# sashajenner/honours

Hardware: AMD Instinct MI355X
Metric: raw-signal MB/s (compress+decompress) (higher is better)
Workload: dtype u16

## Files before the change

### honours_amd/csrc/press_exsplit.hip

```cpp

#include "press_chunk.h"

namespace ph {

__device__ __forceinline__ void quarter_zd(const int16_t *in, uint32_t n, uint32_t ws, int lane, int q,
					   uint4 (&z)[CK], uint32_t &ored)
{
#pragma unroll
	for (int k = 0; k < CK; k++) {
		const uint32_t i0 = ws + k * SUB + lane * 8;
		z[k] = make_uint4(0, 0, 0, 0);
		if (i0 < n)
			z[k] = ld16_stream(in + i0);
	}
	uint32_t carry = 0;
	if (ws > 0 && ws < n)
		carry = (uint32_t) (uint16_t) in[ws - 1] << 16;
	uint32_t o = 0;
	const s16x2 qq = { (short) q, (short) q };
#pragma unroll
	for (int k = 0; k < CK; k++) {
		const uint32_t i0 = ws + k * SUB + lane * 8;
		uint32_t r[4] = { z[k].x, z[k].y, z[k].z, z[k].w };
		if (i0 + 8 > n) {
// ... 422 lines not shown
		unsigned long long mask = __ballot(valid && zv <= 255u);
		while (mask && got < nb) {
			const int l = 63 - __builtin_clzll(mask);
			const uint32_t e = enc[(uint32_t) __builtin_amdgcn_readlane((int) zv, l)];
			const uint32_t len = e >> 24;
			acc = (acc << len) | (e & 0xFFFFFFu);
			got += len;
			mask &= ~(1ull << l);
		}
		pos = pos > 64 ? pos - 64 : 0;
	}
	return got >= nb ? (acc >> (got - nb)) & ((1u << nb) - 1u) : acc;
}


__global__ __launch_bounds__(CWG, HENC_WAVES) void k_huff_encode_chunked(BatchArgs a)
{
	__shared__ uint32_t enc[257];
	__shared__ uint32_t stg_all[4][HSTG];

	enc[threadIdx.x] = a.huff->enc[threadIdx.x];
	if (threadIdx.x == 0)
		enc[256] = 0;
	for (uint32_t i = threadIdx.x; i < 4u * HSTG; i += CWG)
		(&stg_all[0][0])[i] = 0;
	__syncthreads();
	const uint32_t t = blockIdx.x;
	if (t >= uni(a.ctl->nchunks))
		return;
	const int lane = threadIdx.x & 63;
// ... 17 lines not shown
	const uint64_t before = uni64(cb->before);
	if (w == 0 && last) {
		const uint64_t bits = before + q0 + q1 + q2 + q3;
		const uint64_t total = (uint64_t) head + (bits + 7) / 8;
		const uint32_t nbt = (uint32_t) bits & 7u;
		if (total <= cap && nbt) {
			const uint32_t tb = huff_tail_bits(in, n, nbt, enc, lane);
			if (lane == 0)
				payload[bits >> 3] = (uint8_t) tb;
		}
		if (lane == 0)
			a.out_len[d.read] = total <= cap ? total : CFAIL64;
	}
	const uint32_t mybits = w == 0 ? q0 : w == 1 ? q1 : w == 2 ? q2 : q3;
	const uint64_t Bq = before + (w > 0 ? q0 : 0u) + (w > 1 ? q1 : 0u) + (w > 2 ? q2 : 0u);
	if (ws >= n || !mybits || (uint64_t) head + (Bq + mybits + 7) / 8 > cap)
		return;
	const uint32_t nb = (uint32_t) Bq & 7u;
	if (nb) {
		const uint32_t tb = huff_tail_bits(in, ws, nb, enc, lane);
		if (lane == 0)
			stg[0] = tb;
	}
	uint8_t *g = payload + (Bq >> 3);
	uint32_t fill = nb;
	wave_lds_sync();
	static_assert(CK % HENC_G == 0, "a quarter is a whole number of groups");
	uint4 raw[HENC_G];
#pragma unroll
	for (int gi = 0; gi < HENC_G; gi++)
		raw[gi] = sub_load(in, n, ws + gi * SUB + lane * 8);
	uint32_t carry = ws > 0 ? (uint32_t) (uint16_t) in[ws - 1] << 16 : 0u;
// ... 17 lines not shown
			const uint32_t sub0 = ws + (kg + gi) * SUB;
			if (sub0 >= n)
				break;
			const uint32_t i0 = sub0 + lane * 8;
			const uint4 z = sub_zd(cur[gi], n, i0, carry);
			const uint32_t zz[4] = { z.x, z.y, z.z, z.w };
			uint32_t e[8];
			uint32_t lb = 0;
			if (sub0 != 0 && sub0 + SUB <= n && !__ballot(((z.x | z.y | z.z | z.w) & 0xFF00FF00u) != 0)) {
#pragma unroll
				for (int h = 0; h < 8; h++) {
					e[h] = enc[(zz[h >> 1] >> (16 * (h & 1))) & 0xFFu];
					lb += e[h] >> 24;
				}
			} else {
				const uint32_t lowm = low_mask(z, i0, n);
#pragma unroll
				for (int h = 0; h < 8; h++) {
					e[h] = enc[((lowm >> h) & 1u) ? ((zz[h >> 1] >> (16 * (h & 1))) & 0xFFu) : 256u];
					lb += e[h] >> 24;
				}
			}
			const uint32_t inc = wave_incl_scan_dpp(lb);
			const uint32_t tot = (uint32_t) __builtin_amdgcn_readlane((int) inc, 63);
			uint32_t pos = fill + inc - lb;
			if (lb <= 64) {
				uint64_t acc = 0;
				uint32_t o = 0;
#pragma unroll
				for (int h = 0; h < 8; h++) {
// ... 39 lines not shown
			fill = total & 31u;
			wave_lds_sync();
		}
	}
	if (lane == 0) {
		const uint32_t v = stg[0];
		for (uint32_t b = 0; b < (fill >> 3); b++)
			g[b] = (uint8_t) (v >> (8 * b));
	}
}


__global__ __launch_bounds__(256) void k_chunk_prep_meta(const uint64_t *off, const uint64_t *in_off,
							 const ReadMeta *meta, uint32_t nreads, ChunkDesc *chunks,
							 uint64_t *gran, ChunkCtl *ctl, uint32_t max_chunks,
							 uint32_t *out_n, const uint32_t *hread, const uint32_t *ex_pos)
{
	const uint32_t r = blockIdx.x * 256 + threadIdx.x;
	uint32_t n = 0, nch = 0;
	if (r < nreads && !meta[r].status) {
		const uint32_t nex = meta[r].nex;
		n = 1u + meta[r].nlow + nex;
		nch = (n + CHUNK - 1) / CHUNK;
		if (hread && (hread[2 * r + 1] & HUF_FUSED))
			nch = 0;
		else if (hread && nex && (uint64_t) ex_pos[off[r] + nex - 1] + 1 > (uint64_t) meta[r].nlow + nex)
			n = nch = 0;
	}
	const uint32_t inc = scan32(nch, threadIdx.x & 63);
	uint32_t base = 0;
	if ((threadIdx.x & 63) == 63 && inc)
		base = atomicAdd(&ctl->nchunks, inc);
	base = (uint32_t) __builtin_amdgcn_readlane((int) base, 63);
	const uint32_t first = base + inc - nch;
	if (r >= nreads)
		return;
	out_n[r] = n ? n : CFAIL32;
	for (uint32_t j = 0; j < nch && first + j < max_chunks; j++) {
		ChunkDesc d;
		d.sig_off = off[r];
		d.out_base = in_off[r];
		d.n = n;
// ... 63 lines not shown
			if (i == 0) {
				z = zd0;
			} else if (i - 1 == nextpos) {
				z = val[e] & 0xFFFFu;
				e++;
				nextpos = e < nex ? pos[e] : 0xFFFFFFFFu;
			} else {
				z = l < nlow ? low[l] : 0u;
				l++;
			}
			v[h >> 1] |= z << (16 * (h & 1));
		}
	}
}

template <bool HUFF>
__global__ __launch_bounds__(CWG) void k_low_decode_chunked(DecodeArgs a)
{
	__shared__ uint32_t s_ticket;
	__shared__ uint32_t s_wsum[4];
	__shared__ uint32_t s_sbase;
	__shared__ uint16_t s_xl[4][CK][64];
	__shared__ uint32_t s_sub[4][CK];
	__shared__ uint32_t s_cnt[4][CK];
	__shared__ uint32_t s_km[4];

	const int lane = threadIdx.x & 63;
	const int w = (int) uni(threadIdx.x >> 6);
#ifdef DEC_STAMPS
	const uint64_t t_start = __builtin_amdgcn_s_memtime();
#endif
// ... 18 lines not shown
	const ChunkU d = load_chunk(a.chunks + t);
	const uint32_t n = d.n;
	const uint32_t first = d.j * CHUNK;
	const bool last = first + CHUNK >= n;
	const ReadMeta *m = a.meta + d.read;
	const uint32_t nex = uni(m->nex), nlow = uni(m->nlow), zd0 = uni(m->zd0);
	const int q = (int) uni(m->q);
	const uint32_t *pos = a.ex_pos + d.sig_off;
	const uint32_t *val = a.ex_val + d.sig_off;
	const uint8_t *low = HUFF ? a.low + d.sig_off : a.in + d.out_base + uni(m->hdr) + uni(m->seclen);
	int16_t *out = a.sig + d.sig_off;
	const uint32_t ws = first + w * WAVE_SAMPLES;
	const uint32_t nsub = ws >= n ? 0u : min((uint32_t) CK, (n - ws + SUB - 1) / SUB);
	const uint32_t live = (1u << nsub) - 1u;

	const ChunkDesc *dp = a.chunks + t;
	const uint32_t c0 = uni(dp->ecnt[0]), c1 = uni(dp->ecnt[1]), c2 = uni(dp->ecnt[2]), c3 = uni(dp->ecnt[3]);
	const uint32_t ew = w == 0 ? c0 : w == 1 ? c1 : w == 2 ? c2 : c3;
	const uint32_t e_lo = (uint32_t) uni64(dp->ebefore) + (w > 0 ? c0 : 0u) + (w > 1 ? c1 : 0u) + (w > 2 ? c2 : 0u);
	if (nsub) {
		const uint32_t e_hi = e_lo + ew;
		for (uint32_t e = e_lo + lane; e < e_hi; e += 64) {
			const uint32_t k = (pos[e] + 1 - ws) / SUB;
			atomicAdd(&s_cnt[w][k], 1u);
			atomicOr(&s_km[w], 1u << k);
		}
	}
	wave_lds_sync();
	uint32_t kmask = uni(s_km[w]);
	if (ws == 0)
		kmask |= 1u;
	if ((n & 7) && n > ws && n - ws <= WAVE_SAMPLES)
		kmask |= 1u << ((n - 1 - ws) / SUB);
	if (lane < CK) {
// ... 157 lines not shown
static void ex_pass_a(const BatchArgs &a, ExEnt ent, hipStream_t s)
{
	n_pass_a++;
	if (ent == ENT_SHUFF)
		hipLaunchKernelGGL((k_ex_scan_chunked<false, true>), dim3(a.max_chunks), dim3(CWG), 0, s, a);
	else
		hipLaunchKernelGGL((k_ex_scan_chunked<false>), dim3(a.max_chunks), dim3(CWG), 0, s, a);
}

void launch_ex_encode_chunked(const BatchArgs &a, ExFmt fmt, ExEnt ent, hipStream_t s)
{
	if (!a.nreads || !a.max_chunks)
		return;
	ex_encode_prep(a, s);
	ex_pass_a(a, ent, s);
	ex_encode_lists(a, fmt, s);
	ex_encode_streams(a, fmt, ent, s);
}

void ex_packed_sizes(const BatchArgs &a, ExFmt fmt, ExEnt ent, uint64_t *need, hipStream_t s)
{
	const ExStage &st = EX_STAGES[ent];
	launch_ex_sizes(a, fmt, ent, need, s);
	if (st.pay != PAY_STAGED)
		return;
	hipLaunchKernelGGL(k_low_encode_chunked<false>, dim3(a.max_chunks), dim3(CWG), 0, s, a);
	st.press(a, need, s);
}

void ex_packed_streams(const BatchArgs &a, ExFmt fmt, ExEnt ent, hipStream_t s)
{
// ... 2 lines not shown
		return ex_encode_streams(a, fmt, ent, s);
	launch_ex_section(a, fmt, ent, s);
	ktime_begin(0, s);
	st.write_sized(a, s);
	ktime_end(0, s);
}

void launch_ex_encode_packed(const BatchArgs &a, ExFmt fmt, ExEnt ent, const PackArgs &pk, int phases, hipStream_t s)
{
	if (!a.nreads || !a.max_chunks)
		return;
	if (phases & PACK_SIZE) {
		(void) hipMemsetAsync(pk.slot, 0, ((size_t) a.nreads + 1) * 8, s);
		ex_encode_prep(a, s);
		ex_pass_a(a, ent, s);
		ex_encode_lists(a, fmt, s);
		ex_packed_sizes(a, fmt, ent, pk.need, s);
		if (pk.layout) {
			launch_pack_scan(pk, a.nreads, s);
			launch_pack_patch(a, pk.slot, s);
		}
	}
	if (phases & PACK_WRITE)
		ex_packed_streams(a, fmt, ent, s);
}

void launch_ex_prefix_sizes(const BatchArgs &a, ExFmt fmt, ExEnt ent, uint64_t *need, hipStream_t s)
{
	if (!a.nreads || !a.max_chunks || !EX_STAGES[ent].sizes_only)
		return;
	ex_encode_prep(a, s);
	ex_pass_a(a, ent, s);
	ex_encode_lists(a, fmt, s);
	launch_ex_sizes(a, fmt, ent, need, s);
	hipLaunchKernelGGL(k_low_encode_chunked<false>, dim3(a.max_chunks), dim3(CWG), 0, s, a);
	EX_STAGES[ent].press(a, need, s);
}

void ex_encode_lists(const BatchArgs &a, ExFmt fmt, hipStream_t s)
{
	if (fmt == EXF_EXZD) {
		hipLaunchKernelGGL(k_ex_redo_flag, dim3((a.nreads + 255) / 256), dim3(256), 0, s, a);
		hipLaunchKernelGGL((k_ex_scan_chunked<true>), dim3(a.max_chunks), dim3(CWG), 0, s, a);
	}
	hipLaunchKernelGGL(k_ex_prefix, dim3((a.nreads + 3) / 4), dim3(256), 0, s, a, fmt == EXF_EXZD ? 1 : 0);
	hipLaunchKernelGGL(k_ex_list, dim3((a.max_chunks + 3) / 4), dim3(CWG), 0, s, a);
}

void launch_low_encode(const BatchArgs &a, uint64_t *, hipStream_t s)
{
	if (a.zhist)
		hipLaunchKernelGGL(k_low_encode_chunked<true>, dim3(a.max_chunks), dim3(CWG), 0, s, a);
	else
		hipLaunchKernelGGL(k_low_encode_chunked<false>, dim3(a.max_chunks), dim3(CWG), 0, s, a);
}
void launch_shuff_encode(const BatchArgs &a, uint64_t *, hipStream_t s)
{
	hipLaunchKernelGGL(k_huff_encode_chunked, dim3(a.max_chunks), dim3(CWG), 0, s, a);
}

void ex_encode_streams(const BatchArgs &a, ExFmt fmt, ExEnt ent, hipStream_t s)
{
	const ExStage &st = EX_STAGES[ent];
	launch_ex_section(a, fmt, ent, s);
	if (st.low_tmp)
		hipLaunchKernelGGL(k_low_encode_chunked<false>, dim3(a.max_chunks), dim3(CWG), 0, s, a);
	ktime_begin(0, s);
	st.press(a, nullptr, s);
	ktime_end(0, s);
}

void launch_ex_decode_chunked(const DecodeArgs &a, ExFmt fmt, ExEnt ent, hipStream_t s)
{
	const bool huff = EX_STAGES[ent].depress != nullptr;
	if (!a.nreads || !a.max_chunks)
		return;
	launch_ex_parse_huff(a, fmt, ent, s);
	hipLaunchKernelGGL(k_chunk_prep_meta, dim3((a.nreads + 255) / 256), dim3(256), 0, s, a.off, a.in_off,
			   a.meta, a.nreads, a.chunks, a.gran, a.ctl, a.max_chunks, a.out_n,
			   ent == ENT_SHUFF ? (const uint32_t *) a.hread : (const uint32_t *) nullptr, a.ex_pos);
	hipLaunchKernelGGL(k_ex_ranks, dim3((a.max_chunks * 8 + 255) / 256), dim3(256), 0, s, a);
	if (!huff)
		ktime_begin(1, s);
	if (ent == ENT_SHUFF) {
		const uint32_t grid = a.max_chunks < 1024u ? a.max_chunks : 1024u;
		hipLaunchKernelGGL((k_low_decode_chunked<true>), dim3(grid), dim3(CWG), 0, s, a);
	} else if (huff) {
		hipLaunchKernelGGL((k_low_decode_chunked<true>), dim3(a.max_chunks), dim3(CWG), 0, s, a);
	} else {
		hipLaunchKernelGGL((k_low_decode_chunked<false>), dim3(a.max_chunks), dim3(CWG), 0, s, a);
	}
	if (!huff)
		ktime_end(1, s);
}

}
```

### honours_amd/csrc/press_huffman.hip

```cpp

#include "press_internal.h"
#include "press_packed.h"
#include "press_wave.h"
#include <cstddef>
#include <type_traits>

namespace ph {

#ifdef HUF_STAMPS
__device__ unsigned long long g_hstamp[32];
#define HSTAMP_DECL                                             \
	unsigned long long hs_t = __builtin_amdgcn_s_memtime(); \
	unsigned long long hs_acc[8] = { 0, 0, 0, 0, 0, 0, 0, 0 }
#define HSTAMP(i)                                                              \
	do {     \
		__builtin_amdgcn_sched_barrier(0);                             \
		const unsigned long long hs_n = __builtin_amdgcn_s_memtime(); \
		hs_acc[(i) & 7] += hs_n - hs_t;                                \
		hs_t = hs_n;                                                   \
		__builtin_amdgcn_sched_barrier(0);                             \
	} while (0)
#define HSTAMP_FLUSH(base)                                                     \
	do {                                                                   \
		if ((threadIdx.x & 63) == 0)                                   \
// ... 159 lines not shown
}

__device__ __forceinline__ int32_t unzz8(uint32_t z) { return (int32_t) (z >> 1) ^ -(int32_t) (z & 1u); }

typedef __attribute__((address_space(3))) const uint32_t *lds_cu32p;
typedef __attribute__((address_space(3))) const uint16_t *lds_cu16p;
typedef __attribute__((address_space(3))) const uint8_t *lds_cu8p;
typedef __attribute__((address_space(3))) uint8_t *lds_u8p;

struct LenTabs {
	alignas(16) uint32_t alut[1 << HUF_LUT_BITS];
	alignas(16) uint16_t flut[1 << HUF_LUT_BITS];
	alignas(16) uint16_t l2ld[HUF_L2_ENTRIES];
};

template <bool TRIE, int S = 64>
__device__ __forceinline__ uint32_t len_scan(const uint32_t *col_, const LenTabs *tabs, const HuffDev *hd, uint32_t start,
					     uint32_t lim, uint32_t nb, uint32_t &cnt, uint32_t &dsum)
{
	const lds_cu32p col = (lds_cu32p) col_;
	const lds_cu32p alut = (lds_cu32p) tabs->alut;
	const lds_cu16p flut = (lds_cu16p) tabs->flut;
	const lds_cu16p l2ld = (lds_cu16p) tabs->l2ld;
	bool bad = start == HEND;
	uint32_t L = lim < nb ? lim : nb;
	if (bad)
		L = 0;
	auto long_ld = [&](uint32_t e, uint32_t wnd) -> uint32_t {
		if (TRIE && e == 0xFFFFFFFFu) {
			const uint32_t t = trie_code(hd, wnd);
			return t ? (((t >> 24) & 31u) | (((uint32_t) unzz8(t & 0xFFu) & 0xFFu) << 8)) : 0u;
		}
		const uint32_t v = l2ld[(e & 0xFFFu) + ((wnd >> HUF_LUT_BITS) & ((1u << ((e >> 12) & 15u)) - 1u))];
		return v == 0xFFFFu ? 0u : v;
	};
	constexpr uint32_t PB = 30;
	const lds_cu32p colm = col - S;
	uint32_t A = (bad ? 0u : start) + PB;
// ... 55 lines not shown
		const bool fits = pp + tot <= L;
		const bool cut = !fits && pp + len1 > nb;
		if (act && !fail && !cut) {
			p += fits ? tot : len1;
			c += fits ? n : 1u;
			d += fits ? dall : d1;
		}
		if (act && (fail || cut)) {
			bad = true;
			L = 0;
		}
	}
	cnt = c;
	dsum = (uint32_t) d & 0xFFFFu;
	return bad ? HEND : (p >= nb && p < lim ? HEND : p);
}



#ifndef HUF_SYNC_PER_CU
#define HUF_SYNC_PER_CU 2
#endif
#ifndef HUF_RUNUP_EIGHTHS
#define HUF_RUNUP_EIGHTHS 4
#endif
constexpr int WGS = 1024;
constexpr int SYNC_S = 64;

__device__ __forceinline__ uint32_t pack_rec(uint32_t f, uint32_t c, uint32_t d)
{
// ... 258 lines not shown
				atomicAdd(reinterpret_cast<unsigned long long *>(a.hwave + (uint64_t) k * (HT / 64) + (tid >> 6)),
					  (dd << 32) + (unsigned long long) dc);
			if (e8 != old_e) {
				a.hend[g] = (uint8_t) e8;
				const bool more = tid + 1 < HT || !(dp->t_last >> 31);
				next = more && (uint64_t) tid * OWN + OWN < nbits_t;
			}
		}
		list_push(out_list, out_cnt, a.hlist_cap, next, (uint32_t) g + 1, lane);
		if (last && next)
			atomicMin(&a.hmin[dp->read], (uint32_t) g + 1);
	}
}

template <int RU, bool TRIE>
__global__ __launch_bounds__(64) void k_huf_serial(DecodeArgs a)
{
	constexpr int OWN = HufGeo<RU>::OWN, NDW = HufGeo<RU>::NDW, NCOL = HufGeo<RU>::NCOL;
	struct Lds {
		LenTabs tabs;
		uint32_t img[NCOL * 64 + 64];
	};
	__shared__ __attribute__((aligned(16))) Lds lds;
	auto &img = lds.img;

	const uint32_t r = blockIdx.x;
	const uint32_t g0 = uniform(a.hmin[r]);
	if (g0 == 0xFFFFFFFFu)
		return;
	const uint32_t lane = threadIdx.x;
	const uint32_t k0 = uniform(a.hread[2 * r]), nt = uniform(a.hread[2 * r + 1]);
	load_len_tables(a.huff, &lds.tabs, 64);
	uint32_t *col = img + lane;
	const uint64_t gend = (uint64_t) (k0 + nt) * HT;
	for (uint64_t g = g0; g < gend; g++) {
		const uint32_t k = (uint32_t) (g / HT), tid = (uint32_t) (g % HT);
		const HufTile *dp = a.htiles + k;
		const uint32_t nbits_t = uniform(dp->nbits);
		if ((uint64_t) tid * OWN >= nbits_t)
			break;
		const uint32_t pe = uniform((uint32_t) __hip_atomic_load(a.hend + g - 1, __ATOMIC_RELAXED, __HIP_MEMORY_SCOPE_AGENT));
		const uint32_t rec = uniform(__hip_atomic_load(a.hrec + g, __ATOMIC_RELAXED, __HIP_MEMORY_SCOPE_AGENT));
		if ((rec & 0xFFu) == pe)
			continue;
		wave_lds_sync();
		if (lane == 0)
			col_load<NDW>(col, a.in + dp->src, (int32_t) tid * (OWN / 8), 0, (int32_t) ((nbits_t + 7) >> 3));
		wave_lds_sync();
		uint32_t c2, d2;
		const uint32_t e2 = len_scan<TRIE>(col, &lds.tabs, a.huff, (lane || pe == R_END) ? HEND : pe, OWN,
					     clamp_nb((int64_t) nbits_t - (int64_t) tid * OWN), c2, d2);
		if (lane == 0) {
			a.hrec[g] = pack_rec(pe == R_END ? HEND : pe, c2, d2);
			atomicAdd(reinterpret_cast<unsigned long long *>(a.hwave + (uint64_t) k * (HT / 64) + (tid >> 6)),
				  ((unsigned long long) ((d2 - (rec >> 16)) & 0xFFFFu) << 32) +
					  (unsigned long long) (long long) (int32_t) (c2 - ((rec >> 8) & 0xFFu)));
			__hip_atomic_store(a.hend + g, (uint8_t) (e2 == HEND ? R_END : e2 - OWN), __ATOMIC_RELAXED, __HIP_MEMORY_SCOPE_AGENT);
		}
		__builtin_amdgcn_fence(__ATOMIC_RELEASE, "agent");
	}
}

__device__ __forceinline__ uint32_t unzz16(uint32_t z) { return ((z >> 1) ^ (0u - (z & 1u))) & 0xFFFFu; }

__device__ __forceinline__ void keys_below2(const uint32_t *pos, uint32_t nex, uint32_t ka, uint32_t kb, uint32_t &ea, uint32_t &eb)
{
	uint32_t la = 0, lb = 0;
	for (uint32_t step = nex ? 1u << (31 - __builtin_clz(nex)) : 0u; step; step >>= 1) {
		const uint32_t ia = la + step - 1, ib = lb + step - 1;
		const uint32_t pa = ia < nex ? pos[ia] : 0u, pb = ib < nex ? pos[ib] : 0u;
		if (ia < nex && pa - ia < ka)
			la += step;
		if (ib < nex && pb - ib < kb)
			lb += step;
	}
	ea = la;
	eb = lb;
}

template <int RU>
__global__ __launch_bounds__(HT) void k_huf_chain(DecodeArgs a)
{
	constexpr uint32_t UB = 64 * HufGeo<RU>::OWN / 8;
	constexpr uint32_t UPT = HT / 64;
	__shared__ uint32_t s_w[HT / 64], s_wd[HT / 64];
	__shared__ unsigned long long s_cum;
	__shared__ uint32_t s_stop, s_refuse;

	const uint32_t r = blockIdx.x;
	const uint32_t tid = threadIdx.x;
	const uint32_t k0 = uniform(a.hread[2 * r]), nt = uniform(a.hread[2 * r + 1]);
	if (!nt)
		return;
	const uint32_t nu = nt * UPT;
	const uint2 *hw = a.hwave + (uint64_t) k0 * UPT;
	if (tid == 0) {
		s_cum = 0;
		s_stop = 0xFFFFFFFFu;
		s_refuse = 0;
	}
	__syncthreads();
	{
		uint64_t c = 0;
		for (uint32_t u = tid; u < nu; u += HT)
			c += hw[u].x;
		if (c)
			atomicAdd(&s_cum, (unsigned long long) c);
	}
// ... 118 lines not shown
			uint4 *d = reinterpret_cast<uint4 *>(a.hunit + (uint64_t) k0 * UPT + u);
			d[0] = make_uint4((uint32_t) src, (uint32_t) (src >> 32) | (bz << 16), (uint32_t) o0, (uint32_t) (o0 >> 32));
			d[1] = make_uint4(L0, quota | (nbyc << 14) | ((q & 15u) << 26) | (fused ? 1u << 30 : 0u), Ea, Eb - Ea);
		}
		cum += total;
		dcum += dtotal;
		__syncthreads();
	}
	static_assert(HUF_U_QUOTA >= 64u * 255u, "a unit's quota");
	if (tid == 0) {
		a.meta[r].nlow = nlow;
		if (refused)
			a.meta[r].status = 1;
		if (fused)
			a.hread[2 * r + 1] = nt | HUF_FUSED;
	}
}


constexpr uint32_t EMIT_STG = 4096;

template <bool TRIE>
__device__ __forceinline__ void emit_codes(const uint32_t *col_, const uint32_t *lut_, const uint16_t *lut2_,
					   const HuffDev *hd, uint32_t p, uint32_t nmine, uint8_t *wp_)
{
	const lds_cu32p col = (lds_cu32p) col_;
	const lds_cu8p lut = (lds_cu8p) lut_;
	const lds_cu16p lut2 = (lds_cu16p) lut2_;
	auto long_entry = [&](uint32_t e, uint32_t wnd) -> uint32_t {
		if (TRIE && e == 0xFFFFFFFFu) {
// ... 564 lines not shown
namespace ph {
#endif

constexpr int HUF_FIX_LAUNCHES = HUF_FIX_ROUNDS;

template <int RU, bool TRIE>
static void run_huff_decode(const DecodeArgs &a, hipStream_t s)
{
	const uint32_t nt = a.max_htiles ? a.max_htiles : 1;
	const uint32_t ngs = (nt * (HT / 64) + WGS / 64 - 1) / (WGS / 64);
	const uint32_t grid = ngs < HUF_SYNC_PER_CU * 256u ? ngs : HUF_SYNC_PER_CU * 256u;
	const uint32_t nge = (nt * (HT / 64) + WGE / 64 - 1) / (WGE / 64);
	const uint32_t ge = nge < EMIT_PER_CU * 256u ? nge : EMIT_PER_CU * 256u;
	hipLaunchKernelGGL((k_huf_sync<RU, TRIE>), dim3(grid), dim3(WGS), 0, s, a);
	hipLaunchKernelGGL(k_huf_list, dim3((nt * (HT / 64) + LIST_WG - 1) / LIST_WG), dim3(LIST_WG), 0, s, a);
	for (int round = 0; round < HUF_FIX_LAUNCHES; round++)
		hipLaunchKernelGGL((k_huf_fix<RU, TRIE>), dim3(FIX_WG >= 1024 ? 512 : FIX_WG >= 512 ? 768 : 1280), dim3(FIX_WG), 0, s, a, round, round + 1 == HUF_FIX_LAUNCHES ? 1 : 0);
	hipLaunchKernelGGL((k_huf_serial<RU, TRIE>), dim3(a.nreads), dim3(64), 0, s, a);
	hipLaunchKernelGGL(k_huf_chain<RU>, dim3(a.nreads), dim3(HT), 0, s, a);
	hipLaunchKernelGGL((k_huf_emit<RU, TRIE>), dim3(ge), dim3(WGE), 0, s, a);
}

template <int RU>
static void run_huff_decode_t(const DecodeArgs &a, bool trie, hipStream_t s)
{
	if (trie)
		run_huff_decode<RU, true>(a, s);
	else
		run_huff_decode<RU, false>(a, s);
}

void launch_huff_decode(const DecodeArgs &a0, hipStream_t s)
{
	const bool trie = (a0.huf_minlen & HUF_NEEDS_TRIE) != 0;
// ... 14 lines not shown
```

### honours_amd/csrc/press_internal.h

```cpp
#pragma once

#include <hip/hip_runtime.h>
#include <stdint.h>

namespace ph {

enum ExFmt : int {
	EXF_VBE21 = 0,
	EXF_VBBE21 = 1,
	EXF_VBSBE21 = 2,
	EXF_VBSSE21 = 3,
	EXF_EXZD = 4
};
enum ExEnt : int {
	ENT_PLAIN,
	ENT_SHUFF,
	ENT_RC,
	ENT_RCC,
	ENT_RCM,
	ENT_CDF,
	ENT_RICE,
	ENT_DHUF,
	ENT_COUNT
};
// ... 476 lines not shown
	{ ENT_RCM, PAY_CODER, launch_rcm_encode, launch_rcm_decode, true, false, nullptr },
	{ ENT_CDF, PAY_CODER, launch_cdf_encode, launch_cdf_decode, true, false, nullptr },
	{ ENT_RICE, PAY_STAGED, launch_rice_encode, launch_rice_decode, true, true, launch_rice_write_sized },
	{ ENT_DHUF, PAY_STAGED, launch_dhuf_encode, launch_dhuf_decode, true, true, launch_dhuf_write_sized },
};
constexpr bool ex_stages_in_order()
{
	for (int i = 0; i < ENT_COUNT; i++)
		if (EX_STAGES[i].id != i)
			return false;
	return true;
}
static_assert(ex_stages_in_order(), "EX_STAGES[i].id == i");

void ex_encode_prep(const BatchArgs &a, hipStream_t s);
void ex_encode_lists(const BatchArgs &a, ExFmt fmt, hipStream_t s);
void ex_encode_streams(const BatchArgs &a, ExFmt fmt, ExEnt ent, hipStream_t s);
void launch_ex_encode_chunked(const BatchArgs &a, ExFmt fmt, ExEnt ent, hipStream_t s);
void launch_ex_encode_packed(const BatchArgs &a, ExFmt fmt, ExEnt ent, const PackArgs &pk, int phases, hipStream_t s);
void ex_packed_sizes(const BatchArgs &a, ExFmt fmt, ExEnt ent, uint64_t *need, hipStream_t s);
void ex_packed_streams(const BatchArgs &a, ExFmt fmt, ExEnt ent, hipStream_t s);
void launch_ex_prefix_sizes(const BatchArgs &a, ExFmt fmt, ExEnt ent, uint64_t *need, hipStream_t s);
void launch_ex_decode_chunked(const DecodeArgs &a, ExFmt fmt, ExEnt ent, hipStream_t s);
void launch_ex_section(const BatchArgs &a, ExFmt fmt, ExEnt ent, hipStream_t s);
void launch_ex_sizes(const BatchArgs &a, ExFmt fmt, ExEnt ent, uint64_t *need, hipStream_t s);
void launch_ex_parse_huff(const DecodeArgs &a, ExFmt fmt, ExEnt ent, hipStream_t s);
void launch_rcf_raw(const BatchArgs &a, uint8_t *raw, hipStream_t s);
uint64_t train_scratch_bytes(uint32_t max_chunks);
void launch_symbol_counts(const int16_t *sig, const uint64_t *off, const uint32_t *n, uint32_t nreads, uint64_t *counts,
			  void *chunks, uint32_t *nchunks, uint32_t max_chunks, uint32_t grid, hipStream_t s);

// ... 8 lines not shown
```

### honours_amd/csrc/press_sections.hip

```cpp

#include <stdlib.h>

#include "press_internal.h"
#include "press_packed.h"

namespace ph {

constexpr uint64_t FAIL64 = ~0ull;


__device__ __forceinline__ void put8(uint8_t *p, uint32_t v) { p[0] = (uint8_t) v; }
__device__ __forceinline__ void put16(uint8_t *p, uint32_t v) { p[0] = (uint8_t) v; p[1] = (uint8_t) (v >> 8); }
__device__ __forceinline__ void put32(uint8_t *p, uint32_t v)
{
	p[0] = (uint8_t) v; p[1] = (uint8_t) (v >> 8); p[2] = (uint8_t) (v >> 16); p[3] = (uint8_t) (v >> 24);
}
__device__ __forceinline__ uint32_t get16(const uint8_t *p) { return (uint32_t) p[0] | ((uint32_t) p[1] << 8); }
__device__ __forceinline__ uint32_t get32(const uint8_t *p)
{
	return (uint32_t) p[0] | ((uint32_t) p[1] << 8) | ((uint32_t) p[2] << 16) | ((uint32_t) p[3] << 24);
}

__device__ __forceinline__ uint32_t svb32_nbytes(uint32_t v)
{
// ... 181 lines not shown
	uint8_t *p = out;
	if (l0) {
		if (fmt == EXF_EXZD) {
			p[0] = 0;
			put32(p + 1, n);
			put32(p + 5, 0);
			p[9] = (uint8_t) mq;
			put16(p + 10, zd0);
		} else {
			put16(p, zd0);
		}
		put32(p + hdr, nex);
	}
	p += hdr + 4;
	if (fmt == EXF_VBE21) {
	} else if (nex == 1) {
		if (l0) {
			put32(p, pos[0]);
			if (fmt == EXF_EXZD)
				put32(p + 4, val[0] - 256u);
			else
				put16(p + 4, val[0] - 256u);
		}
	} else if (nex > 1) {
		if (l0)
			put32(p, len_pos);
		p += 4;
		if (fmt == EXF_VBBE21)
			w_bitpack_write(p, nex, bits_pos, pos, nullptr, lane, s_buf);
		else
// ... 53 lines not shown
			const ChunkBits *cb = a.cbits + last;
			const uint64_t bits = cb->before + cb->q[0] + cb->q[1] + cb->q[2] + cb->q[3];
			size = hdr + seclen + 4 + (bits + 7) / 8;
		} else if (pay == PAY_CODER) {
			size += RC_PACK_SLACK;
		} else if (pay == PAY_STAGED) {
			size = hdr + seclen;
		}
		if ((pay == PAY_SHUFF || pay == PAY_CODER) && fmt != EXF_VBE21 && seclen > 65535)
			size = FAIL64;
		if (fmt == EXF_EXZD && hdr + seclen + nlow > 2ull * n + 1024)
			size = FAIL64;
	}
	if (lane == 0)
		need[r] = size;
}

__global__ __launch_bounds__(64) void k_ex_fill_vbe21(BatchArgs a)
{
	const uint32_t r = blockIdx.x;
	const ReadMeta *m = a.meta + r;
	if (m->status)
		return;
	const uint32_t nex = m->nex;
	const uint64_t o0 = a.off[r];
	const uint32_t *pos = a.ex_pos + o0;
	const uint32_t *val = a.ex_val + o0;
	uint8_t *p = a.out + a.out_off[r] + m->hdr + 4;
	for (uint32_t k = threadIdx.x; k < nex; k += 64) {
		put32(p + 4ull * k, pos[k]);
		put16(p + 4ull * nex + 2ull * k, val[k]);
	}
}


struct BlockReader {
	const uint8_t *in;
	uint32_t len;
	int kind;
	uint32_t bits;
	uint32_t dptr;
	bool bad;
};

__device__ __forceinline__ BlockReader block_open(const uint8_t *in, uint32_t len, uint32_t nex, int kind)
{
	BlockReader b = { in, len, kind, 0, 0, false };
// ... 140 lines not shown
				before = prev_last;
			if (act) {
				pos[k] = pk;
				val[k] = (v + 256u) & 0xFFFFu;
				if (pk >= cap - 1 || (k && pk <= before))
					wrong = true;
			}
			carry += (uint32_t) __builtin_amdgcn_readlane((int) inc, 63);
			prev_last = (uint32_t) __builtin_amdgcn_readlane((int) pk, 63);
		}
		if (__ballot(wrong || bp.bad || bv.bad))
			return;
		last = prev_last;
		seclen += 8ull + lp + lv;
	}
	if (!l0)
		return;
	m->nex = nex;
	m->seclen = (uint32_t) seclen;
	uint64_t nlow;
	const bool rest = pay == PAY_CODER || pay == PAY_STAGED;
	if (rest) {
		nlow = (uint64_t) cap - 1 - nex;
	} else if (pay == PAY_SHUFF) {
		const uint64_t hl = len - hdr - seclen;
		if (hl <= 4)
			return;
		const uint8_t *h = in + hdr + seclen;
		nlow = ((uint32_t) h[0] << 24) | ((uint32_t) h[1] << 16) | ((uint32_t) h[2] << 8) | h[3];
	} else {
		nlow = len - hdr - seclen;
	}
	if (1ull + nlow + nex > lim)
		return;
	if (!rest && nex && fmt != EXF_VBE21 && (uint64_t) last + 1 > (uint64_t) nlow + nex)
		return;
	m->nlow = (uint32_t) nlow;
	m->status = 0;
}

__global__ __launch_bounds__(64) void k_ex_parse_fill_vbe21(DecodeArgs a)
{
	const uint32_t r = blockIdx.x;
	ReadMeta *m = a.meta + r;
	if (m->status)
		return;
	const uint32_t nex = m->nex;
	const uint32_t cap = a.nsamp[r];
	const uint64_t o0 = a.off[r];
	uint32_t *pos = a.ex_pos + o0;
	uint32_t *val = a.ex_val + o0;
	const uint8_t *p = a.in + a.in_off[r] + m->hdr + 4;
	bool bad = false;
	for (uint32_t k = threadIdx.x; k < nex; k += 64) {
		const uint32_t pk = get32(p + 4ull * k);
		pos[k] = pk;
		val[k] = get16(p + 4ull * nex + 2ull * k);
		if (pk >= cap - 1 || (k && pk <= get32(p + 4ull * (k - 1))))
			bad = true;
		if (k == nex - 1 && (uint64_t) pk + 1 > (uint64_t) m->nlow + nex)
			bad = true;
	}
	if (__ballot(bad) && threadIdx.x == 0)
		m->status = 1;
}


void launch_ex_section(const BatchArgs &a, ExFmt fmt, ExEnt ent, hipStream_t s)
{
	hipLaunchKernelGGL(k_ex_section, dim3(a.nreads), dim3(64), 0, s, a, fmt, EX_STAGES[ent].pay);
	if (fmt == EXF_VBE21)
		hipLaunchKernelGGL(k_ex_fill_vbe21, dim3(a.nreads), dim3(64), 0, s, a);
}

void launch_ex_sizes(const BatchArgs &a, ExFmt fmt, ExEnt ent, uint64_t *need, hipStream_t s)
{
	hipLaunchKernelGGL(k_ex_sizes, dim3(a.nreads), dim3(64), 0, s, a, fmt, EX_STAGES[ent].pay, need);
}

void launch_ex_parse_huff(const DecodeArgs &a, ExFmt fmt, ExEnt ent, hipStream_t s)
{
	hipLaunchKernelGGL(k_ex_parse, dim3(a.nreads), dim3(64), 0, s, a, fmt, EX_STAGES[ent].pay);
	if (fmt == EXF_VBE21)
		hipLaunchKernelGGL(k_ex_parse_fill_vbe21, dim3(a.nreads), dim3(64), 0, s, a);
	if (EX_STAGES[ent].depress) {
		ktime_begin(1, s);
		EX_STAGES[ent].depress(a, s);
		ktime_end(1, s);
	}
}

}
```

### honours_amd/csrc/press_svb.hip

```cpp

#include "press_chunk.h"

namespace ph {


template <bool DEC, bool KEY2, bool EXACT = false>
__global__ __launch_bounds__(256) void k_chunk_prep(const uint64_t *off, const uint32_t *nsamp,
						    const uint64_t *slot_off, const uint64_t *in_len,
						    uint32_t nreads, ChunkDesc *chunks, uint64_t *gran,
						    ChunkCtl *ctl, uint32_t max_chunks, uint64_t *out_len,
						    uint32_t *out_n, uint32_t *first_chunk, ReadMeta *meta = nullptr,
						    const uint8_t *in = nullptr, uint32_t hdr = 0, uint8_t *out = nullptr,
						    const uint64_t *need = nullptr, uint64_t out_cap = 0)
{
	static_assert(!EXACT || !DEC, "the exact slots are press's");
	const uint32_t r = blockIdx.x * 256 + threadIdx.x;
	uint32_t n = 0, nch = 0;
	if (r < nreads) {
		n = nsamp[r];
		nch = (n + CHUNK - 1) / CHUNK;
	}
	const uint32_t inc = scan32(nch, threadIdx.x & 63);
	uint32_t base = 0;
	if ((threadIdx.x & 63) == 63 && inc)
// ... 1074 lines not shown
	ktime_end(1, s);
}

template <bool KEY2, bool S5>
static void run_recode(const DecodeArgs &d, const BatchArgs &p, ExFmt fmt, ExEnt ent, const PackArgs *pk, int phases, uint32_t bits,
		       hipStream_t s)
{
	if (phases & PACK_SIZE) {
		svb_decode_front<KEY2, S5>(d, s);
		launch_recode_counts(d.out_n, const_cast<uint32_t *>(p.nsamp), d.nreads, s);
		if (pk)
			(void) hipMemsetAsync(pk->slot, 0, ((size_t) p.nreads + 1) * 8, s);
		ex_encode_prep(p, s);
		const FuseArgs f = { p.chunks, p.first_chunk, p.cbits, p.meta, p.huff, nullptr, nullptr, degrade_h2(bits), degrade_m2(bits) };
		run_decode_fused<KEY2, S5>(d, f, ent, bits, s);
		ex_encode_lists(p, fmt, s);
		if (pk) {
			ex_packed_sizes(p, fmt, ent, pk->need, s);
			launch_pack_scan_refused(*pk, d.out_n, d.nreads, s);
			if (pk->layout)
				launch_pack_patch(p, pk->slot, s);
		}
	}
	if (phases & PACK_WRITE) {
		if (pk)
			ex_packed_streams(p, fmt, ent, s);
		else
			ex_encode_streams(p, fmt, ent, s);
	}
}

// ... 26 lines not shown
```

Before: 874,700.

## Fuse exception list writing, serial walk, and chunk prep into neighboring kernels

Removes several small per-read kernels. The VBE21 exception-section fill is folded into the section and parse kernels. The exception list for the SHUFF path is written directly by the Huffman encoder. The serial Huffman walk and chunk-descriptor creation move into k_huf_chain, and decoding computes exception ranks by binary search instead of relying on k_chunk_prep_meta/k_ex_ranks. It also shrinks the grid for the later fix rounds. The aim is to cut launch overhead and redundant global passes, at the cost of extra work and LDS inside the encode and chain kernels, plus more complex synchronisation (agent-scope fences) and atomics on ctl-1.

Result: faster. 884,200 (median of 5 runs) (+1.1%).

```diff
diff --git a/honours_amd/csrc/press_exsplit.hip b/honours_amd/csrc/press_exsplit.hip
--- a/honours_amd/csrc/press_exsplit.hip
+++ b/honours_amd/csrc/press_exsplit.hip
@@ -460,6 +460,44 @@
 }
 
 
+__device__ __forceinline__ void xsec_put(uint8_t *xsec, uint32_t nex, uint32_t p, uint32_t position, uint32_t value)
+{
+	const uint16_t v16 = (uint16_t) value;
+	__builtin_memcpy(xsec + 4ull * p, &position, 4);
+	__builtin_memcpy(xsec + 4ull * nex + 2ull * p, &v16, 2);
+}
+
+__device__ __forceinline__ uint32_t xsec_subtile(uint8_t *xsec, uint32_t nex, uint32_t rank, const uint4 &z, uint32_t em, uint32_t i0)
+{
+	const uint32_t c = __popc(em);
+	const uint32_t inc = wave_incl_scan_dpp(c);
+	if (em) {
+		const uint32_t zz[4] = { z.x, z.y, z.z, z.w };
+		uint32_t p = rank + inc - c;
+#pragma unroll
+		for (int h = 0; h < 8; h++) {
+			if ((em >> h) & 1u) {
+				xsec_put(xsec, nex, p, i0 + h - 1, (zz[h >> 1] >> (16 * (h & 1))) & 0xFFFFu);
+				p++;
+			}
+		}
+	}
+	return (uint32_t) __builtin_amdgcn_readlane((int) inc, 63);
+}
+
+__device__ __noinline__ void xsec_quarter(uint8_t *xsec, uint32_t nex, uint32_t rank, const int16_t *in, uint32_t n, uint32_t ws,
+					  uint32_t km, int lane)
+{
+	for (uint32_t mm = km; mm; mm &= mm - 1) {
+		const uint32_t sub0 = ws + (uint32_t) __builtin_ctz(mm) * SUB;
+		const uint32_t i0 = sub0 + lane * 8;
+		uint32_t carry = sub0 ? (uint32_t) (uint16_t) in[sub0 - 1] << 16 : 0u;
+		const uint4 z = sub_zd(sub_load(in, n, i0), n, i0, carry);
+		rank += xsec_subtile(xsec, nex, rank, z, exc_mask(z, i0), i0);
+	}
+}
+
+template <bool XSEC>
 __global__ __launch_bounds__(CWG, HENC_WAVES) void k_huff_encode_chunked(BatchArgs a)
 {
 	__shared__ uint32_t enc[257];
@@ -507,8 +545,19 @@
 	}
 	const uint32_t mybits = w == 0 ? q0 : w == 1 ? q1 : w == 2 ? q2 : q3;
 	const uint64_t Bq = before + (w > 0 ? q0 : 0u) + (w > 1 ? q1 : 0u) + (w > 2 ? q2 : 0u);
-	if (ws >= n || !mybits || (uint64_t) head + (Bq + mybits + 7) / 8 > cap)
-		return;
+	uint8_t *xsec = nullptr;
+	uint32_t nex = 0, xrank = 0;
+	if (XSEC) {
+		const uint32_t c0 = uni(dp->ecnt[0]), c1 = uni(dp->ecnt[1]), c2 = uni(dp->ecnt[2]);
+		xsec = a.out + d.out_base + uni(m->hdr) + 4;
+		nex = uni(m->nex);
+		xrank = (uint32_t) uni64(dp->ebefore) + (w > 0 ? c0 : 0u) + (w > 1 ? c1 : 0u) + (w > 2 ? c2 : 0u);
+	}
+	if (ws >= n || !mybits || (uint64_t) head + (Bq + mybits + 7) / 8 > cap) {
+		if (XSEC && ws < n && uni(dp->kmask[w]))
+			xsec_quarter(xsec, nex, xrank, in, n, ws, uni(dp->kmask[w]), lane);
+		return;
+	}
 	const uint32_t nb = (uint32_t) Bq & 7u;
 	if (nb) {
 		const uint32_t tb = huff_tail_bits(in, ws, nb, enc, lane);
@@ -556,6 +605,11 @@
 					lb += e[h] >> 24;
 				}
 			} else {
+				if (XSEC) {
+					const uint32_t em = exc_mask(z, i0);
+					if (__ballot(em != 0))
+						xrank += xsec_subtile(xsec, nex, xrank, z, em, i0);
+				}
 				const uint32_t lowm = low_mask(z, i0, n);
 #pragma unroll
 				for (int h = 0; h < 8; h++) {
@@ -625,18 +679,13 @@
 __global__ __launch_bounds__(256) void k_chunk_prep_meta(const uint64_t *off, const uint64_t *in_off,
 							 const ReadMeta *meta, uint32_t nreads, ChunkDesc *chunks,
 							 uint64_t *gran, ChunkCtl *ctl, uint32_t max_chunks,
-							 uint32_t *out_n, const uint32_t *hread, const uint32_t *ex_pos)
+							 uint32_t *out_n)
 {
 	const uint32_t r = blockIdx.x * 256 + threadIdx.x;
 	uint32_t n = 0, nch = 0;
 	if (r < nreads && !meta[r].status) {
-		const uint32_t nex = meta[r].nex;
-		n = 1u + meta[r].nlow + nex;
+		n = 1u + meta[r].nlow + meta[r].nex;
 		nch = (n + CHUNK - 1) / CHUNK;
-		if (hread && (hread[2 * r + 1] & HUF_FUSED))
-			nch = 0;
-		else if (hread && nex && (uint64_t) ex_pos[off[r] + nex - 1] + 1 > (uint64_t) meta[r].nlow + nex)
-			n = nch = 0;
 	}
 	const uint32_t inc = scan32(nch, threadIdx.x & 63);
 	uint32_t base = 0;
@@ -730,7 +779,7 @@
 	}
 }
 
-template <bool HUFF>
+template <bool HUFF, bool RANKS = false>
 __global__ __launch_bounds__(CWG) void k_low_decode_chunked(DecodeArgs a)
 {
 	__shared__ uint32_t s_ticket;
@@ -779,10 +828,20 @@
 	const uint32_t nsub = ws >= n ? 0u : min((uint32_t) CK, (n - ws + SUB - 1) / SUB);
 	const uint32_t live = (1u << nsub) - 1u;
 
-	const ChunkDesc *dp = a.chunks + t;
-	const uint32_t c0 = uni(dp->ecnt[0]), c1 = uni(dp->ecnt[1]), c2 = uni(dp->ecnt[2]), c3 = uni(dp->ecnt[3]);
-	const uint32_t ew = w == 0 ? c0 : w == 1 ? c1 : w == 2 ? c2 : c3;
-	const uint32_t e_lo = (uint32_t) uni64(dp->ebefore) + (w > 0 ? c0 : 0u) + (w > 1 ? c1 : 0u) + (w > 2 ? c2 : 0u);
+	uint32_t ew, e_lo;
+	if (RANKS) {
+		auto below = [&](uint32_t s) {
+			const uint32_t upto = s < n ? s : n;
+			return lower_bound_dev(pos, nex, upto ? upto - 1 : 0);
+		};
+		e_lo = uni(below(ws));
+		ew = uni(below(ws + WAVE_SAMPLES)) - e_lo;
+	} else {
+		const ChunkDesc *dp = a.chunks + t;
+		const uint32_t c0 = uni(dp->ecnt[0]), c1 = uni(dp->ecnt[1]), c2 = uni(dp->ecnt[2]), c3 = uni(dp->ecnt[3]);
+		ew = w == 0 ? c0 : w == 1 ? c1 : w == 2 ? c2 : c3;
+		e_lo = (uint32_t) uni64(dp->ebefore) + (w > 0 ? c0 : 0u) + (w > 1 ? c1 : 0u) + (w > 2 ? c2 : 0u);
+	}
 	if (nsub) {
 		const uint32_t e_hi = e_lo + ew;
 		for (uint32_t e = e_lo + lane; e < e_hi; e += 64) {
@@ -970,7 +1029,7 @@
 		return;
 	ex_encode_prep(a, s);
 	ex_pass_a(a, ent, s);
-	ex_encode_lists(a, fmt, s);
+	ex_encode_lists(a, fmt, ent, s);
 	ex_encode_streams(a, fmt, ent, s);
 }
 
@@ -1003,7 +1062,7 @@
 		(void) hipMemsetAsync(pk.slot, 0, ((size_t) a.nreads + 1) * 8, s);
 		ex_encode_prep(a, s);
 		ex_pass_a(a, ent, s);
-		ex_encode_lists(a, fmt, s);
+		ex_encode_lists(a, fmt, ent, s);
 		ex_packed_sizes(a, fmt, ent, pk.need, s);
 		if (pk.layout) {
 			launch_pack_scan(pk, a.nreads, s);
@@ -1020,20 +1079,21 @@
 		return;
 	ex_encode_prep(a, s);
 	ex_pass_a(a, ent, s);
-	ex_encode_lists(a, fmt, s);
+	ex_encode_lists(a, fmt, ent, s);
 	launch_ex_sizes(a, fmt, ent, need, s);
 	hipLaunchKernelGGL(k_low_encode_chunked<false>, dim3(a.max_chunks), dim3(CWG), 0, s, a);
 	EX_STAGES[ent].press(a, need, s);
 }
 
-void ex_encode_lists(const BatchArgs &a, ExFmt fmt, hipStream_t s)
+void ex_encode_lists(const BatchArgs &a, ExFmt fmt, ExEnt ent, hipStream_t s)
 {
 	if (fmt == EXF_EXZD) {
 		hipLaunchKernelGGL(k_ex_redo_flag, dim3((a.nreads + 255) / 256), dim3(256), 0, s, a);
 		hipLaunchKernelGGL((k_ex_scan_chunked<true>), dim3(a.max_chunks), dim3(CWG), 0, s, a);
 	}
 	hipLaunchKernelGGL(k_ex_prefix, dim3((a.nreads + 3) / 4), dim3(256), 0, s, a, fmt == EXF_EXZD ? 1 : 0);
-	hipLaunchKernelGGL(k_ex_list, dim3((a.max_chunks + 3) / 4), dim3(CWG), 0, s, a);
+	if (!ex_lists_in_encoder(fmt, ent))
+		hipLaunchKernelGGL(k_ex_list, dim3((a.max_chunks + 3) / 4), dim3(CWG), 0, s, a);
 }
 
 void launch_low_encode(const BatchArgs &a, uint64_t *, hipStream_t s)
@@ -1045,7 +1105,7 @@
 }
 void launch_shuff_encode(const BatchArgs &a, uint64_t *, hipStream_t s)
 {
-	hipLaunchKernelGGL(k_huff_encode_chunked, dim3(a.max_chunks), dim3(CWG), 0, s, a);
+	hipLaunchKernelGGL(k_huff_encode_chunked<false>, dim3(a.max_chunks), dim3(CWG), 0, s, a);
 }
 
 void ex_encode_streams(const BatchArgs &a, ExFmt fmt, ExEnt ent, hipStream_t s)
@@ -1055,7 +1115,10 @@
 	if (st.low_tmp)
 		hipLaunchKernelGGL(k_low_encode_chunked<false>, dim3(a.max_chunks), dim3(CWG), 0, s, a);
 	ktime_begin(0, s);
-	st.press(a, nullptr, s);
+	if (ex_lists_in_encoder(fmt, ent))
+		hipLaunchKernelGGL(k_huff_encode_chunked<true>, dim3(a.max_chunks), dim3(CWG), 0, s, a);
+	else
+		st.press(a, nullptr, s);
 	ktime_end(0, s);
 }
 
@@ -1065,16 +1128,17 @@
 	if (!a.nreads || !a.max_chunks)
 		return;
 	launch_ex_parse_huff(a, fmt, ent, s);
+	if (ent == ENT_SHUFF) {
+		const uint32_t grid = a.max_chunks < 1024u ? a.max_chunks : 1024u;
+		hipLaunchKernelGGL((k_low_decode_chunked<true, true>), dim3(grid), dim3(CWG), 0, s, a);
+		return;
+	}
 	hipLaunchKernelGGL(k_chunk_prep_meta, dim3((a.nreads + 255) / 256), dim3(256), 0, s, a.off, a.in_off,
-			   a.meta, a.nreads, a.chunks, a.gran, a.ctl, a.max_chunks, a.out_n,
-			   ent == ENT_SHUFF ? (const uint32_t *) a.hread : (const uint32_t *) nullptr, a.ex_pos);
+			   a.meta, a.nreads, a.chunks, a.gran, a.ctl, a.max_chunks, a.out_n);
 	hipLaunchKernelGGL(k_ex_ranks, dim3((a.max_chunks * 8 + 255) / 256), dim3(256), 0, s, a);
 	if (!huff)
 		ktime_begin(1, s);
-	if (ent == ENT_SHUFF) {
-		const uint32_t grid = a.max_chunks < 1024u ? a.max_chunks : 1024u;
-		hipLaunchKernelGGL((k_low_decode_chunked<true>), dim3(grid), dim3(CWG), 0, s, a);
-	} else if (huff) {
+	if (huff) {
 		hipLaunchKernelGGL((k_low_decode_chunked<true>), dim3(a.max_chunks), dim3(CWG), 0, s, a);
 	} else {
 		hipLaunchKernelGGL((k_low_decode_chunked<false>), dim3(a.max_chunks), dim3(CWG), 0, s, a);
diff --git a/honours_amd/csrc/press_huffman.hip b/honours_amd/csrc/press_huffman.hip
--- a/honours_amd/csrc/press_huffman.hip
+++ b/honours_amd/csrc/press_huffman.hip
@@ -197,14 +197,15 @@
 	alignas(16) uint16_t l2ld[HUF_L2_ENTRIES];
 };
 
-template <bool TRIE, int S = 64>
-__device__ __forceinline__ uint32_t len_scan(const uint32_t *col_, const LenTabs *tabs, const HuffDev *hd, uint32_t start,
-					     uint32_t lim, uint32_t nb, uint32_t &cnt, uint32_t &dsum)
-{
+template <bool TRIE, int S, bool GT>
+__device__ __forceinline__ uint32_t len_scan_at(const uint32_t *col_, const uint32_t *alut_, const uint16_t *flut_, const uint16_t *l2ld_,
+						const HuffDev *hd, uint32_t start, uint32_t lim, uint32_t nb, uint32_t &cnt, uint32_t &dsum)
+{
+	typedef typename std::conditional<GT, const uint16_t *, lds_cu16p>::type cu16p;
 	const lds_cu32p col = (lds_cu32p) col_;
-	const lds_cu32p alut = (lds_cu32p) tabs->alut;
-	const lds_cu16p flut = (lds_cu16p) tabs->flut;
-	const lds_cu16p l2ld = (lds_cu16p) tabs->l2ld;
+	const lds_cu32p alut = (lds_cu32p) alut_;
+	const cu16p flut = (cu16p) flut_;
+	const cu16p l2ld = (cu16p) l2ld_;
 	bool bad = start == HEND;
 	uint32_t L = lim < nb ? lim : nb;
 	if (bad)
@@ -290,6 +291,13 @@
 	cnt = c;
 	dsum = (uint32_t) d & 0xFFFFu;
 	return bad ? HEND : (p >= nb && p < lim ? HEND : p);
+}
+
+template <bool TRIE, int S = 64>
+__device__ __forceinline__ uint32_t len_scan(const uint32_t *col_, const LenTabs *tabs, const HuffDev *hd, uint32_t start,
+					     uint32_t lim, uint32_t nb, uint32_t &cnt, uint32_t &dsum)
+{
+	return len_scan_at<TRIE, S, false>(col_, tabs->alut, tabs->flut, tabs->l2ld, hd, start, lim, nb, cnt, dsum);
 }
 
 
@@ -578,24 +586,11 @@
 }
 
 template <int RU, bool TRIE>
-__global__ __launch_bounds__(64) void k_huf_serial(DecodeArgs a)
-{
-	constexpr int OWN = HufGeo<RU>::OWN, NDW = HufGeo<RU>::NDW, NCOL = HufGeo<RU>::NCOL;
-	struct Lds {
-		LenTabs tabs;
-		uint32_t img[NCOL * 64 + 64];
-	};
-	__shared__ __attribute__((aligned(16))) Lds lds;
-	auto &img = lds.img;
-
-	const uint32_t r = blockIdx.x;
-	const uint32_t g0 = uniform(a.hmin[r]);
-	if (g0 == 0xFFFFFFFFu)
-		return;
-	const uint32_t lane = threadIdx.x;
-	const uint32_t k0 = uniform(a.hread[2 * r]), nt = uniform(a.hread[2 * r + 1]);
-	load_len_tables(a.huff, &lds.tabs, 64);
-	uint32_t *col = img + lane;
+__device__ __forceinline__ void huf_serial_walk(const DecodeArgs &a, uint32_t g0, uint32_t k0, uint32_t nt, uint32_t *col,
+						const uint32_t *alut, uint32_t lane)
+{
+	constexpr int OWN = HufGeo<RU>::OWN, NDW = HufGeo<RU>::NDW;
+	const HuffDev *hd = a.huff;
 	const uint64_t gend = (uint64_t) (k0 + nt) * HT;
 	for (uint64_t g = g0; g < gend; g++) {
 		const uint32_t k = (uint32_t) (g / HT), tid = (uint32_t) (g % HT);
@@ -609,11 +604,11 @@
 			continue;
 		wave_lds_sync();
 		if (lane == 0)
-			col_load<NDW>(col, a.in + dp->src, (int32_t) tid * (OWN / 8), 0, (int32_t) ((nbits_t + 7) >> 3));
+			col_load<NDW, 1>(col, a.in + dp->src, (int32_t) tid * (OWN / 8), 0, (int32_t) ((nbits_t + 7) >> 3));
 		wave_lds_sync();
 		uint32_t c2, d2;
-		const uint32_t e2 = len_scan<TRIE>(col, &lds.tabs, a.huff, (lane || pe == R_END) ? HEND : pe, OWN,
-					     clamp_nb((int64_t) nbits_t - (int64_t) tid * OWN), c2, d2);
+		const uint32_t e2 = len_scan_at<TRIE, 1, true>(col, alut, hd->flut, hd->l2ld, hd, (lane || pe == R_END) ? HEND : pe, OWN,
+							       clamp_nb((int64_t) nbits_t - (int64_t) tid * OWN), c2, d2);
 		if (lane == 0) {
 			a.hrec[g] = pack_rec(pe == R_END ? HEND : pe, c2, d2);
 			atomicAdd(reinterpret_cast<unsigned long long *>(a.hwave + (uint64_t) k * (HT / 64) + (tid >> 6)),
@@ -642,11 +637,43 @@
 	eb = lb;
 }
 
-template <int RU>
-__global__ __launch_bounds__(HT) void k_huf_chain(DecodeArgs a)
+__device__ __forceinline__ void chain_finish(const DecodeArgs &a, uint32_t r, bool ok, bool fused, uint32_t nlow, uint32_t nex,
+					     const uint32_t *pos)
+{
+	uint32_t n = ok ? 1u + nlow + nex : 0u;
+	if (n && !fused && nex && (uint64_t) pos[nex - 1] + 1 > (uint64_t) nlow + nex)
+		n = 0;
+	a.out_n[r] = n ? n : 0xFFFFFFFFu;
+	if (!n || fused)
+		return;
+	const uint32_t nch = (n + CHUNK - 1) / CHUNK;
+	const uint32_t first = atomicAdd(&(a.ctl - 1)->nchunks, nch);
+	for (uint32_t j = 0; j < nch && first + j < a.max_chunks; j++) {
+		ChunkDesc d;
+		d.sig_off = a.off[r];
+		d.out_base = a.in_off[r];
+		d.n = n;
+		d.j = j;
+		d.read = r;
+		d.cap_ok = 1;
+		d.ebefore = 0;
+		d.ecnt[0] = d.ecnt[1] = d.ecnt[2] = d.ecnt[3] = 0;
+		d.kmask[0] = d.kmask[1] = d.kmask[2] = d.kmask[3] = 0;
+		a.chunks[first + j] = d;
+		a.gran[first + j] = 0;
+	}
+}
+
+template <int RU, bool TRIE>
+__global__ __launch_bounds__(HT, 8) void k_huf_chain(DecodeArgs a)
 {
 	constexpr uint32_t UB = 64 * HufGeo<RU>::OWN / 8;
 	constexpr uint32_t UPT = HT / 64;
+	struct WalkLds {
+		alignas(16) uint32_t alut[1 << HUF_LUT_BITS];
+		uint32_t img[HufGeo<RU>::NCOL + 2];
+	};
+	__shared__ __attribute__((aligned(16))) WalkLds s_walk;
 	__shared__ uint32_t s_w[HT / 64], s_wd[HT / 64];
 	__shared__ unsigned long long s_cum;
 	__shared__ uint32_t s_stop, s_refuse;
@@ -654,8 +681,27 @@
 	const uint32_t r = blockIdx.x;
 	const uint32_t tid = threadIdx.x;
 	const uint32_t k0 = uniform(a.hread[2 * r]), nt = uniform(a.hread[2 * r + 1]);
-	if (!nt)
+	if (!nt) {
+		if (tid == 0) {
+			const ReadMeta *m = a.meta + r;
+			chain_finish(a, r, m->status == 0, false, m->nlow, m->nex, a.ex_pos + a.off[r]);
+		}
 		return;
+	}
+	const uint32_t g0 = uniform(a.hmin[r]);
+	if (g0 != 0xFFFFFFFFu) {
+		const uint4 *s4 = reinterpret_cast<const uint4 *>(a.huff->alut);
+		uint4 *d4 = reinterpret_cast<uint4 *>(s_walk.alut);
+		for (uint32_t i = tid; i < (1u << HUF_LUT_BITS) / 4; i += HT)
+			d4[i] = s4[i];
+		__syncthreads();
+		if (tid < 64) {
+			huf_serial_walk<RU, TRIE>(a, g0, k0, nt, s_walk.img + 1, s_walk.alut, tid);
+			__builtin_amdgcn_fence(__ATOMIC_RELEASE, "agent");
+		}
+		__syncthreads();
+		__builtin_amdgcn_fence(__ATOMIC_ACQUIRE, "agent");
+	}
 	const uint32_t nu = nt * UPT;
 	const uint2 *hw = a.hwave + (uint64_t) k0 * UPT;
 	if (tid == 0) {
@@ -804,6 +850,7 @@
 			a.meta[r].status = 1;
 		if (fused)
 			a.hread[2 * r + 1] = nt | HUF_FUSED;
+		chain_finish(a, r, !refused, fused, nlow, nex, pos);
 	}
 }
 
@@ -1398,10 +1445,10 @@
 	const uint32_t ge = nge < EMIT_PER_CU * 256u ? nge : EMIT_PER_CU * 256u;
 	hipLaunchKernelGGL((k_huf_sync<RU, TRIE>), dim3(grid), dim3(WGS), 0, s, a);
 	hipLaunchKernelGGL(k_huf_list, dim3((nt * (HT / 64) + LIST_WG - 1) / LIST_WG), dim3(LIST_WG), 0, s, a);
+	const uint32_t gfix = FIX_WG >= 1024 ? 512 : FIX_WG >= 512 ? 768 : 1280;
 	for (int round = 0; round < HUF_FIX_LAUNCHES; round++)
-		hipLaunchKernelGGL((k_huf_fix<RU, TRIE>), dim3(FIX_WG >= 1024 ? 512 : FIX_WG >= 512 ? 768 : 1280), dim3(FIX_WG), 0, s, a, round, round + 1 == HUF_FIX_LAUNCHES ? 1 : 0);
-	hipLaunchKernelGGL((k_huf_serial<RU, TRIE>), dim3(a.nreads), dim3(64), 0, s, a);
-	hipLaunchKernelGGL(k_huf_chain<RU>, dim3(a.nreads), dim3(HT), 0, s, a);
+		hipLaunchKernelGGL((k_huf_fix<RU, TRIE>), dim3(round < 2 ? gfix : round == 2 ? gfix / 4 : gfix / 16), dim3(FIX_WG), 0, s, a, round, round + 1 == HUF_FIX_LAUNCHES ? 1 : 0);
+	hipLaunchKernelGGL((k_huf_chain<RU, TRIE>), dim3(a.nreads), dim3(HT), 0, s, a);
 	hipLaunchKernelGGL((k_huf_emit<RU, TRIE>), dim3(ge), dim3(WGE), 0, s, a);
 }
 
diff --git a/honours_amd/csrc/press_internal.h b/honours_amd/csrc/press_internal.h
--- a/honours_amd/csrc/press_internal.h
+++ b/honours_amd/csrc/press_internal.h
@@ -514,7 +514,8 @@
 static_assert(ex_stages_in_order(), "EX_STAGES[i].id == i");
 
 void ex_encode_prep(const BatchArgs &a, hipStream_t s);
-void ex_encode_lists(const BatchArgs &a, ExFmt fmt, hipStream_t s);
+void ex_encode_lists(const BatchArgs &a, ExFmt fmt, ExEnt ent, hipStream_t s);
+constexpr bool ex_lists_in_encoder(ExFmt fmt, ExEnt ent) { return fmt == EXF_VBE21 && ent == ENT_SHUFF; }
 void ex_encode_streams(const BatchArgs &a, ExFmt fmt, ExEnt ent, hipStream_t s);
 void launch_ex_encode_chunked(const BatchArgs &a, ExFmt fmt, ExEnt ent, hipStream_t s);
 void launch_ex_encode_packed(const BatchArgs &a, ExFmt fmt, ExEnt ent, const PackArgs &pk, int phases, hipStream_t s);
diff --git a/honours_amd/csrc/press_sections.hip b/honours_amd/csrc/press_sections.hip
--- a/honours_amd/csrc/press_sections.hip
+++ b/honours_amd/csrc/press_sections.hip
@@ -219,6 +219,10 @@
 	}
 	p += hdr + 4;
 	if (fmt == EXF_VBE21) {
+		for (uint32_t k = lane; k < nex && pay != PAY_SHUFF; k += 64) {
+			put32(p + 4ull * k, pos[k]);
+			put16(p + 4ull * nex + 2ull * k, val[k]);
+		}
 	} else if (nex == 1) {
 		if (l0) {
 			put32(p, pos[0]);
@@ -302,23 +306,6 @@
 	}
 	if (lane == 0)
 		need[r] = size;
-}
-
-__global__ __launch_bounds__(64) void k_ex_fill_vbe21(BatchArgs a)
-{
-	const uint32_t r = blockIdx.x;
-	const ReadMeta *m = a.meta + r;
-	if (m->status)
-		return;
-	const uint32_t nex = m->nex;
-	const uint64_t o0 = a.off[r];
-	const uint32_t *pos = a.ex_pos + o0;
-	const uint32_t *val = a.ex_val + o0;
-	uint8_t *p = a.out + a.out_off[r] + m->hdr + 4;
-	for (uint32_t k = threadIdx.x; k < nex; k += 64) {
-		put32(p + 4ull * k, pos[k]);
-		put16(p + 4ull * nex + 2ull * k, val[k]);
-	}
 }
 
 
@@ -489,10 +476,10 @@
 		last = prev_last;
 		seclen += 8ull + lp + lv;
 	}
-	if (!l0)
-		return;
-	m->nex = nex;
-	m->seclen = (uint32_t) seclen;
+	if (l0) {
+		m->nex = nex;
+		m->seclen = (uint32_t) seclen;
+	}
 	uint64_t nlow;
 	const bool rest = pay == PAY_CODER || pay == PAY_STAGED;
 	if (rest) {
@@ -510,42 +497,29 @@
 		return;
 	if (!rest && nex && fmt != EXF_VBE21 && (uint64_t) last + 1 > (uint64_t) nlow + nex)
 		return;
+	bool bad = false;
+	if (fmt == EXF_VBE21) {
+		for (uint32_t k = lane; k < nex; k += 64) {
+			const uint32_t pk = get32(p + 4ull * k);
+			pos[k] = pk;
+			val[k] = get16(p + 4ull * nex + 2ull * k);
+			if (pk >= cap - 1 || (k && pk <= get32(p + 4ull * (k - 1))))
+				bad = true;
+			if (k == nex - 1 && (uint64_t) pk + 1 > (uint64_t) (uint32_t) nlow + nex)
+				bad = true;
+		}
+		bad = __ballot(bad) != 0;
+	}
+	if (!l0)
+		return;
 	m->nlow = (uint32_t) nlow;
-	m->status = 0;
-}
-
-__global__ __launch_bounds__(64) void k_ex_parse_fill_vbe21(DecodeArgs a)
-{
-	const uint32_t r = blockIdx.x;
-	ReadMeta *m = a.meta + r;
-	if (m->status)
-		return;
-	const uint32_t nex = m->nex;
-	const uint32_t cap = a.nsamp[r];
-	const uint64_t o0 = a.off[r];
-	uint32_t *pos = a.ex_pos + o0;
-	uint32_t *val = a.ex_val + o0;
-	const uint8_t *p = a.in + a.in_off[r] + m->hdr + 4;
-	bool bad = false;
-	for (uint32_t k = threadIdx.x; k < nex; k += 64) {
-		const uint32_t pk = get32(p + 4ull * k);
-		pos[k] = pk;
-		val[k] = get16(p + 4ull * nex + 2ull * k);
-		if (pk >= cap - 1 || (k && pk <= get32(p + 4ull * (k - 1))))
-			bad = true;
-		if (k == nex - 1 && (uint64_t) pk + 1 > (uint64_t) m->nlow + nex)
-			bad = true;
-	}
-	if (__ballot(bad) && threadIdx.x == 0)
-		m->status = 1;
+	m->status = bad ? 1 : 0;
 }
 
 
 void launch_ex_section(const BatchArgs &a, ExFmt fmt, ExEnt ent, hipStream_t s)
 {
 	hipLaunchKernelGGL(k_ex_section, dim3(a.nreads), dim3(64), 0, s, a, fmt, EX_STAGES[ent].pay);
-	if (fmt == EXF_VBE21)
-		hipLaunchKernelGGL(k_ex_fill_vbe21, dim3(a.nreads), dim3(64), 0, s, a);
 }
 
 void launch_ex_sizes(const BatchArgs &a, ExFmt fmt, ExEnt ent, uint64_t *need, hipStream_t s)
@@ -556,8 +530,6 @@
 void launch_ex_parse_huff(const DecodeArgs &a, ExFmt fmt, ExEnt ent, hipStream_t s)
 {
 	hipLaunchKernelGGL(k_ex_parse, dim3(a.nreads), dim3(64), 0, s, a, fmt, EX_STAGES[ent].pay);
-	if (fmt == EXF_VBE21)
-		hipLaunchKernelGGL(k_ex_parse_fill_vbe21, dim3(a.nreads), dim3(64), 0, s, a);
 	if (EX_STAGES[ent].depress) {
 		ktime_begin(1, s);
 		EX_STAGES[ent].depress(a, s);
diff --git a/honours_amd/csrc/press_svb.hip b/honours_amd/csrc/press_svb.hip
--- a/honours_amd/csrc/press_svb.hip
+++ b/honours_amd/csrc/press_svb.hip
@@ -1112,7 +1112,7 @@
 		ex_encode_prep(p, s);
 		const FuseArgs f = { p.chunks, p.first_chunk, p.cbits, p.meta, p.huff, nullptr, nullptr, degrade_h2(bits), degrade_m2(bits) };
 		run_decode_fused<KEY2, S5>(d, f, ent, bits, s);
-		ex_encode_lists(p, fmt, s);
+		ex_encode_lists(p, fmt, ent, s);
 		if (pk) {
 			ex_packed_sizes(p, fmt, ent, pk->need, s);
 			launch_pack_scan_refused(*pk, d.out_n, d.nreads, s);
```
